# real-world-cryprography/APSU

Hardware: AMD Instinct MI355X
Metric: sender query-eval ms (ComputePowers + all BinBundles + gather), 16M-4096 params (lower is better)
Workload: dtype u64; 1 GPU; 16M-4096: n=8192, 4 bundle indices x 7 BinBundles (degrees [1303, 170]), 6 source -> 72 target powers, ps_low_degree=44; db_bytes_rank0=5459379072, binbundles_rank0=28, parallelism=binbundle-shard x1

## Files before the change

### apsu_amd/csrc/dev_consts.cpp

```cpp
#include "dev_consts.h"
#include "eval_plan.h"
#include "mac_core.h"

#include <algorithm>
#include <cstdint>
#include <cstdlib>
#include <cstring>
#include <stdexcept>
#include <string>
#include <utility>

namespace apsu_he {

uint32_t packed_row_bits(u64 q)
{
    const int bits = 64 - __builtin_clzll(q);
    for (u32 c = (u32)std::max(bits, 32); c < 64; c++) {
        u32 g = 2 * c, r = 32;
        while (r) { const u32 t2 = g % r; g = r; r = t2; }
        if ((32 - g) + 2 * c <= 128) return c;
    }
    return 64;
}

// ... 195 lines not shown
        DevLevel &d = dc.key_level[0];
        std::memset(&d, 0, sizeof(d));
        d.L = hp.K;
        for (int j = 0; j < hp.K; j++) d.q[j] = k.q[j];
    }
    for (u64 q : hp.key_q) {
        dc.max_multiple.push_back(~(u64)0 - (~(u64)0 % q) - 1);
        dc.row_bits.push_back(packed_row_bits(q));
    }
}

DeviceConstants build_device_constants(const HeParams &hp)
{
    DeviceConstants dc;
    build_transform_tables(hp, dc);
    build_levels(hp, dc);
    build_key(hp, dc);
    dc.data_primes_narrow = true;
    for (u64 q : hp.key_q) dc.data_primes_narrow = dc.data_primes_narrow && ntt_is_narrow(q, hp.logn);
    dc.ext_primes_narrow = dc.data_primes_narrow;
    for (u64 m : hp.aux_primes) dc.ext_primes_narrow = dc.ext_primes_narrow && ntt_is_narrow(m, hp.logn);
    dc.unlift_exact = hp.batching && hp.key_q[0] / 2 >= hp.t && hp.key_q[0] > 2 * hp.t;
    return dc;
}

EngineSwitches read_switches()
{
    EngineSwitches s;
    auto flag = [](const char *name, auto &out) { if (const char *v = std::getenv(name)) out = std::atoi(v) != 0; };
    auto size = [](const char *name, size_t &out) { if (const char *v = std::getenv(name)) out = std::strtoull(v, nullptr, 10); };
    flag("APSU_HE_SPLIT", s.two_stream_default);
    flag("APSU_HE_MAC_KARA", s.mac_kara);
    flag("APSU_HE_EVAL_SIDE", s.eval_side);
    flag("APSU_HE_PACKED_ROWS", s.packed_rows);
    flag("APSU_HE_EVAL_PER_TERM", s.force_per_term);
    flag("APSU_HE_SEED_EXPAND_HOST", s.seed_expand_host);
    flag("APSU_HE_FUSE_TAIL", s.fuse_tail);
    size("APSU_HE_EVAL_WS_BYTES", s.eval_ws_bytes);
    size("APSU_HE_ARENA_BYTES", s.arena_bytes);
    size("APSU_HE_NTT_LATENCY_LIMBS", s.ntt_latency_limbs);
    size("APSU_HE_SEED_REJ_CAP", s.seed_rej_cap);
    return s;
}

}
```

### apsu_amd/csrc/dev_consts.h

```cpp
#pragma once
#include <cstddef>
#include <vector>

#include "modmath.h"
#include "ntt_core.h"
#include "ntt_form.h"
#include "params.h"

namespace apsu_he {

constexpr int EW_T = 256;
constexpr int DMAXL = 8;
constexpr int DMAXB = DMAXL + 2;
constexpr int DMAXE = DMAXL + DMAXB;
constexpr u32 SEED_REJ_CAP = 8192;

struct ShoupConst { u64 w, wq; };

struct DevLevel {
    int L, nB, nBsk, E;
    Mod q[DMAXL];
    Mod bsk[DMAXB];
    Mod ext[DMAXE];
    u64 t;
// ... 65 lines not shown
}
inline NttTable make_ntt_table(const NttTablesHost &t, int logn, const TwPair *fwd, const TwPair *dit, const TwPair *scale)
{
    NttTable tb = make_ntt_table(t.mod.value, logn);
    tb.ninv = t.ninv;
    tb.ninv_q = t.ninv_q;
    tb.fwd = fwd;
    tb.dit = dit;
    tb.scale = scale;
    return tb;
}

struct DeviceConstants {
    std::vector<TwPair> tw;
    std::vector<NttTable> tabs;
    std::vector<ShoupConst> fin, drop, mdtw;
    std::vector<DevLevel> levels;
    DevKey key;
    std::vector<int> map_ext, map_ext_fin, map_ks, map_ksacc, map_ksacc_raw, map_ct;
    std::vector<DevLevel> key_level;
    std::vector<u64> max_multiple;
    bool data_primes_narrow = false;
    bool ext_primes_narrow = false;
    bool unlift_exact = false;
    std::vector<u32> row_bits;
    void relocate(const TwPair *tw_base, const ShoupConst *fin_base, const ShoupConst *drop_base, const ShoupConst *mdtw_base);
};
DeviceConstants build_device_constants(const HeParams &hp);

struct EngineSwitches {
    static constexpr size_t ARENA_AUTO = ~(size_t)0;
    int two_stream_default = -1;
    bool eval_side = true;
    bool packed_rows = true;
    size_t eval_ws_bytes = (size_t)6 << 30;
    size_t arena_bytes = ARENA_AUTO;
    bool force_per_term = false;
    int mac_kara = -1;
    bool seed_expand_host = false;
    size_t seed_rej_cap = SEED_REJ_CAP;
    bool fuse_tail = true;
    size_t ntt_latency_limbs = NTT_FORM_AUTO;
};
EngineSwitches read_switches();

}
```

### apsu_amd/csrc/emu/rules.cpp

```cpp
#include <cstring>
#include <set>
#include <stdexcept>
#include <vector>

#include "emu_common.h"
#include "bundle_layout.h"
#include "dev_consts.h"
#include "eval_plan.h"
#include "params.h"
#include "powers_dag.h"
#include "powers_sched.h"
#include "sched_policy.h"

using namespace apsu_he;

extern "C" {

const char *emu_last_error() { return g_err.c_str(); }

int emu_plan_walk(unsigned bits, int split_mode)
{
    WalkState s{};
    s.recycled = bits & 1; s.last_use_set = bits & 2; s.last_use_done = bits & 4; s.high_async = bits & 8; s.split_ok = bits & 16;
    s.prof_on = bits & 32; s.pipe_cp = bits & 64; s.force_pipe = bits & 128; s.inputs_ready = bits & 256; s.on_device = bits & 512;
    s.device_busy = bits & 1024; s.split_mode = split_mode;
    const WalkPlan p = plan_walk(s);
    return p.walk | (p.main_waits_high_ready ? 4 : 0) | (p.side_waits_last_use ? 8 : 0) | (p.side_waits_main ? 16 : 0) | (p.consumes_last_use ? 32 : 0);
}
int emu_pick_pooled_buffer(const unsigned char *entries, int count, int inputs_ready)
{
    std::vector<PoolEntryState> st(count);
    for (int i = 0; i < count; i++) st[i] = PoolEntryState{ (entries[i] & 1) != 0, (entries[i] & 2) != 0, (entries[i] & 4) != 0 };
    return pick_pooled_buffer(st.data(), st.size(), inputs_ready != 0);
}

int emu_plan_eval(unsigned bits, int low, int high, int L, int nB, uint32_t l, uint64_t q_last, uint64_t q_widest, int Bs, int max_terms)
{
    EvalState s{};
    s.low = low; s.high = high; s.L = L; s.nB = nB; s.l = l; s.q_last = q_last; s.q_widest = q_widest; s.Bs = Bs; s.max_terms = max_terms;
    s.high_in_flight = bits & 1; s.eval_side = bits & 2; s.prof_on = bits & 4; s.force_per_term = bits & 8; s.fuse_tensor = bits & 16;
    s.fuse_tail = bits & 32; s.lane2 = bits & 64; s.on_lane0 = bits & 128;
    const EvalPlan p = plan_eval(s);
    return (int)p.i0_fast | p.need_vlast << 1 | p.raw_drop << 2 | p.raw_i0 << 3 | p.fused_drop << 4 | p.summed << 5 | p.side << 6 | p.side_i0 << 7 |
           p.wait_high_ready << 8 | p.fuse_tensor << 9 | p.fuse_tail << 10 | p.cf << 11 | p.i0 << 13;
}
int emu_behz_unrolled(int L, int nB) { return behz_unrolled(L, nB); }

int emu_bundle_layout(uint32_t ps_low_degree, uint32_t degree, int first_chain_idx, uint64_t *out, int cap, uint32_t *where)
{
    try {
        const BundleLayout y = bundle_layout(ps_low_degree, degree, first_chain_idx);
        std::vector<u64> v{ y.use_ps, y.H, y.r, (u64)y.pt_level, y.ntt_count, y.lifted_count, y.runs.size() };
        for (const BundleRun &r : y.runs) v.insert(v.end(), { r.d0, r.count, (u64)r.kind, r.first_slot });
        for (size_t i = 0; i < v.size() && (int)i < cap; i++) out[i] = v[i];
        for (uint32_t d = 0; where && d <= degree; d++) { where[2 * d] = (uint32_t)y.where(d).kind; where[2 * d + 1] = y.where(d).slot; }
        return (int)v.size();
    } catch (const std::invalid_argument &e) { g_err = e.what(); return -1; }
}

void emu_ntt_form(int logn, int kind, size_t limbs, size_t latency_limbs, int narrow, int *out)
{
    const NttForm f = ntt_form(logn, (NttKind)kind, limbs, latency_limbs, narrow != 0);
    out[0] = f.threads; out[1] = f.coeffs_per_lane; out[2] = f.min_waves; out[3] = f.split;
}

int emu_params_info(const char *json, uint64_t *out, int cap)
{
    try {
        PSUParams p = PSUParams::Load(json);
        HeParams hp = HeParams::FromPSUParams(p);
        std::vector<u64> v;
        v.push_back(hp.n); v.push_back(hp.K); v.push_back(hp.first_chain_idx); v.push_back(hp.t);
        for (u64 q : hp.key_q) v.push_back(q);
        for (int j = 0; j < hp.K; j++) v.push_back(hp.ntt[j].psi);
        const LevelConstants &lv = hp.level[hp.first_chain_idx];
        v.push_back(lv.nB); v.push_back(lv.m_sk); v.push_back(lv.gamma);
        for (u64 b : lv.B) v.push_back(b);
// ... 166 lines not shown
```

### apsu_amd/csrc/engine.cpp

```cpp
#include "engine_impl.h"

namespace apsu_he {

void throw_hip(hipError_t e, const char *file, int line)
{
    throw HipError(std::string("HIP error: ") + hipGetErrorString(e) + " at " + file + ":" + std::to_string(line));
}

void DevBuf::alloc(size_t bytes)
{
    release();
    if (!bytes) return;
    HIP_CHECK(hipMalloc(&p_, bytes));
    bytes_ = bytes;
}
void DevBuf::release()
{
    if (p_) (void)hipFree(p_);
    p_ = nullptr;
    bytes_ = 0;
}

int Powers::slot_of(uint32_t bundle_idx) const
{
// ... 2 lines not shown
}

Engine::Engine(const HeParams &hp, const PSUParams *psu, int device) : hp_(hp), device_(device)
{
    if (psu) { psu_ = *psu; has_psu_ = true; }
    if (sw_.seed_rej_cap < 1 || sw_.seed_rej_cap > SEED_REJ_CAP) throw std::invalid_argument("APSU_HE_SEED_REJ_CAP outside 1 .. 8192");
    int ndev = 0;
    hipError_t e = hipGetDeviceCount(&ndev);
    if (e != hipSuccess || ndev == 0)
        throw HipError("no HIP device available: the query-evaluation engine has no CPU fallback");
    if (device < 0 || device >= ndev) throw std::invalid_argument("device index out of range");
    DeviceConstants dc = build_device_constants(hp_);
    data_primes_narrow_ = dc.data_primes_narrow;
    ext_primes_narrow_ = dc.ext_primes_narrow;
    unlift_exact_ = dc.unlift_exact;
    key_level_ = dc.key_level;
    max_multiple_ = dc.max_multiple;
    if (hp_.logn == 15) fuse_tensor_ = false;
    packed_rows_ = sw_.packed_rows && hp_.using_keyswitching;
    struct Restore { int prev = -1; ~Restore() { if (prev >= 0) (void)hipSetDevice(prev); } } restore;
    { int cur = -1; if (hipGetDevice(&cur) == hipSuccess && cur != device) restore.prev = cur; }
    HIP_CHECK(hipSetDevice(device));
    HIP_CHECK(hipStreamCreateWithFlags(&st_, hipStreamNonBlocking));
    {
        int least = 0, greatest = 0;
        HIP_CHECK(hipDeviceGetStreamPriorityRange(&least, &greatest));
        HIP_CHECK(hipStreamCreateWithPriority(&lanes_[1].st, hipStreamNonBlocking, greatest));
        HIP_CHECK(hipStreamCreateWithPriority(&lanes_[2].st, hipStreamNonBlocking, greatest));
    }
    HIP_CHECK(hipEventCreateWithFlags(&ev_main_, hipEventDisableTiming));
    HIP_CHECK(hipEventCreateWithFlags(&ev_fork_, hipEventDisableTiming));
    HIP_CHECK(hipEventCreateWithFlags(&ev_side_, hipEventDisableTiming));
    HIP_CHECK(hipEventCreateWithFlags(&ev_intt_, hipEventDisableTiming));

    auto each = [&](auto f) {
        f(d_tw_, dc.tw); f(d_tabs_, dc.tabs); f(d_fin_, dc.fin); f(d_drop_, dc.drop); f(d_levels_, dc.levels);
        f(d_map_ext_, dc.map_ext); f(d_map_ext_fin_, dc.map_ext_fin); f(d_map_ks_, dc.map_ks); f(d_map_ksacc_, dc.map_ksacc);
        f(d_map_ksacc_raw_, dc.map_ksacc_raw); f(d_map_ct_, dc.map_ct); f(d_mdtw_, dc.mdtw);
    };
    each([](DevBuf &b, const auto &v) { b.alloc(v.size() * sizeof(v[0])); });
    d_key_.alloc(sizeof(DevKey));
    dc.relocate(reinterpret_cast<const TwPair *>(d_tw_.p()), reinterpret_cast<const ShoupConst *>(d_fin_.p()),
                reinterpret_cast<const ShoupConst *>(d_drop_.p()), reinterpret_cast<const ShoupConst *>(d_mdtw_.p()));
    each([](DevBuf &b, const auto &v) { if (b.p()) HIP_CHECK(hipMemcpy(b.p(), v.data(), b.bytes(), hipMemcpyHostToDevice)); });
    HIP_CHECK(hipMemcpy(d_key_.p(), &dc.key, sizeof(DevKey), hipMemcpyHostToDevice));
    if (hp_.batching) {
        d_slot_map_.alloc(hp_.slot_map.size() * sizeof(uint32_t));
        HIP_CHECK(hipMemcpy(d_slot_map_.p(), hp_.slot_map.data(), hp_.slot_map.size() * sizeof(uint32_t), hipMemcpyHostToDevice));
    }
    if (has_psu_) {
        auto targets = create_powers_set(psu_.query_params.ps_low_degree, psu_.table_params.max_items_per_bin);
        if (!dag_.configure(psu_.query_params.query_powers, targets))
            throw std::invalid_argument("failed to configure PowersDag");
        const uint32_t ps = psu_.query_params.ps_low_degree;
        PowersScheds scheds = powers_scheds(dag_, ps);
        split_ok_ = scheds.split_ok;
        sched_ = std::move(scheds.all); sched_low_ = std::move(scheds.low); sched_high_ = std::move(scheds.high);
        sizes_ = power_sizes(sched_, hp_.using_keyswitching, dag_.depth());
        result_polys_ = apsu_he::result_polys(sizes_, ps, hp_.using_keyswitching, psu_.table_params.max_items_per_bin);
    }
    const size_t init = sw_.arena_bytes != EngineSwitches::ARENA_AUTO ? sw_.arena_bytes : 4096 * hp_.n * sizeof(u64);
    arena_.alloc(init);
    lanes_[1].arena.alloc(std::max<size_t>(init / 4, (size_t)1 << 20));
    lanes_[2].arena.alloc((size_t)1 << 20);
    stage_bytes_ = 4u << 20;
    HIP_CHECK(hipHostMalloc(&stage_, stage_bytes_));
    HIP_CHECK(hipHostMalloc(reinterpret_cast<void **>(&bad_source_), BAD_SLOTS * sizeof(unsigned)));
    for (int i = 0; i < BAD_SLOTS; i++) bad_source_[i] = 0;
}

Engine::~Engine()
{
    int cur = -1;
    const bool switched = hipGetDevice(&cur) == hipSuccess && cur != device_ && hipSetDevice(device_) == hipSuccess;
    struct Back { bool on; int dev; ~Back() { if (on) (void)hipSetDevice(dev); } } back{ switched, cur };
    if (st_) (void)hipStreamSynchronize(st_);
    for (Lane &l : lanes_) if (l.st) (void)hipStreamSynchronize(l.st);
    powers_pool_.clear();
    if (st_) (void)hipStreamDestroy(st_);
    for (Lane &l : lanes_) if (l.st) (void)hipStreamDestroy(l.st);
    for (hipEvent_t e : inflight_) if (e) (void)hipEventDestroy(e);
    for (PhaseSpan &sp : phase_spans_) for (hipEvent_t e : { sp.a, sp.b, sp.b2 }) if (e) (void)hipEventDestroy(e);
    for (hipEvent_t e : phase_pool_) if (e) (void)hipEventDestroy(e);
    for (hipEvent_t e : { query_start_, query_end_ }) if (e) (void)hipEventDestroy(e);
    if (ev_main_) (void)hipEventDestroy(ev_main_);
    for (OpClock &c : clock_) c.evs.release();
    if (ev_fork_) (void)hipEventDestroy(ev_fork_);
    if (ev_side_) (void)hipEventDestroy(ev_side_);
    if (ev_intt_) (void)hipEventDestroy(ev_intt_);
    if (stage_) (void)hipHostFree(stage_);
    if (bad_source_) (void)hipHostFree(bad_source_);
    if (wire_pinned_) (void)hipHostFree(wire_pinned_);
}

void Engine::wire_stage(size_t bytes, u64 **device, u64 **pinned)
{
    Enter g(this);
    if (wire_dev_.bytes() < bytes) { sync(); wire_dev_.alloc(bytes + bytes / 4); }
    if (wire_pinned_bytes_ < bytes) {
        sync();
        if (wire_pinned_) (void)hipHostFree(wire_pinned_);
        wire_pinned_ = nullptr; wire_pinned_bytes_ = 0;
        HIP_CHECK(hipHostMalloc(&wire_pinned_, bytes + bytes / 4));
        wire_pinned_bytes_ = bytes + bytes / 4;
    }
    *device = wire_dev_.u();
    *pinned = static_cast<u64 *>(wire_pinned_);
}

void Engine::sync()
{
    counters_[C_HOST_SYNC]++;
    HIP_CHECK(hipStreamSynchronize(st_));
    for (Lane &l : lanes_) if (l.st) HIP_CHECK(hipStreamSynchronize(l.st));
    if (prof_on_) prof_collect();
}

bool Engine::bad_source_pending(int slot, bool take)
{
    if (!bad_source_) return false;
    const unsigned v = *const_cast<volatile unsigned *>(bad_source_ + slot);
    if (v == bad_reported_[slot]) return false;
// ... 510 lines not shown
```

### apsu_amd/csrc/engine.h

```cpp
#pragma once
#include <hip/hip_runtime.h>

#include <functional>
#include <memory>
#include <mutex>
#include <string>
#include <vector>

#include "device.h"
#include "params.h"
#include "db_place.h"
#include "db_compact.h"
#include "bulk_place.h"
#include "powers_dag.h"
#include "powers_sched.h"
#include "bundle_layout.h"

namespace apsu_he {

struct HipError : std::runtime_error { using std::runtime_error::runtime_error; };

class DevBuf {
public:
    DevBuf() = default;
// ... 247 lines not shown
    const int *map_ksacc_raw(int chain_idx) const { return reinterpret_cast<const int *>(d_map_ksacc_raw_.p()) + chain_idx * (DMAXL + 1); }

    void d_ntt(u64 *data, size_t count, const int *modmap, int period, bool inverse, bool narrow);
    void d_ntt_ct(u64 *data, size_t polys, int chain_idx, bool inverse) { d_ntt(data, polys * (chain_idx + 1), map_ct(), chain_idx + 1, inverse, data_primes_narrow_); }
    bool d_relinearize(u64 *ct3, size_t ct_stride, int batch, const RelinKeys &rk, int chain_idx, u64 *ext_out = nullptr, int n_ext = 0,
                       u64 **defer_moddown = nullptr);
    void check_level(int chain_idx) const;
    void check_tier1_residues(const u64 *ct, size_t polys, int chain_idx, const char *what) const;
    void d_multiply_sized(const u64 *ea, int sa, const u64 *eb, int sb, u64 *out, int chain_idx);
    std::unique_ptr<Powers> compute_powers_nks(const uint32_t *bundle_indices, int nb, const u64 *const *src, bool on_device);
    void eval_bundles_nks(const Bundle *const *bundles, int count, const Powers &pw, const u64 *const *masks, bool masks_on_device,
                          u64 *out, bool out_on_device, u64 *const *out_rows);
    PowerSizes sizes_;
    uint32_t result_polys_ = 2;

    HeParams hp_;
    const EngineSwitches sw_ = read_switches();
    PSUParams psu_;
    bool has_psu_ = false;
    PowersDag dag_;
    int device_ = 0;
    hipStream_t st_ = nullptr;
    std::mutex mu_;

    DevBuf d_tabs_, d_tw_, d_levels_, d_key_, d_map_ct_, d_map_ext_, d_map_ext_fin_, d_map_ks_, d_map_ksacc_, d_map_ksacc_raw_, d_fin_, d_drop_, d_mdtw_;
    DevBuf arena_;
    size_t arena_off_ = 0;
    struct Lane { hipStream_t st = nullptr; DevBuf arena; size_t off = 0, job_seq = 0; };
    Lane lanes_[3];
    int cur_lane_ = 0, overflow_lane_ = 0;
    void switch_lane(int lane);
    hipEvent_t ev_main_ = nullptr;
    hipEvent_t ev_fork_ = nullptr, ev_side_ = nullptr, ev_intt_ = nullptr;
    bool inputs_ready_ = false;
    bool pipe_cp_ = true;
    bool force_pipe_ = false;
    bool data_primes_narrow_ = false;
    bool ext_primes_narrow_ = false;
    bool async_results_ = false;
    std::vector<hipEvent_t> inflight_;
    size_t inflight_head_ = 0, inflight_count_ = 0;
    int max_inflight_ = 2;
    void throttle_inflight();
    void mark_inflight();
    static constexpr int BAD_SLOTS = 16;
    unsigned *bad_source_ = nullptr;
    unsigned bad_reported_[BAD_SLOTS] = {};
    uint32_t query_seq_ = 0;
    void check_sources();
    void check_sources(const Powers &pw);
    bool bad_source_pending(int slot, bool take);
    void *stage_ = nullptr;
    size_t stage_bytes_ = 0, stage_off_ = 0;
    struct JobWay { DevBuf buf; std::vector<unsigned char> host; uint64_t stamp = 0; };
    struct JobSlot { JobWay way[4]; };
    uint64_t job_stamp_ = 0;
    std::vector<JobSlot> job_slots_;
    size_t job_seq_ = 0, job_seq_base_ = 0;
    std::vector<std::unique_ptr<Powers>> powers_pool_;
public:
    void recycle_powers(std::unique_ptr<Powers> p);
private:
    std::vector<DevBuf> retired_;
    uint64_t counters_[C_COUNT] = {};
    std::mutex wire_mu_;
    DevBuf wire_dev_;
// ... 1 lines not shown
    size_t wire_pinned_bytes_ = 0;

    PowersSched sched_, sched_low_, sched_high_;
    void mask_generate_impl(uint32_t count, u64 *masks_dev, u64 *values_host, u64 *blocks_host, const std::function<void(u64 *, size_t)> &fill);
    bool fuse_tensor_ = true;
    bool tier1_device_ = false;
    void tier1_done() { if (!tier1_device_ || prof_on_) sync(); }
    bool packed_rows_ = true;
    BundleLayout layout_of(uint32_t degree) const { return bundle_layout(psu_.query_params.ps_low_degree, degree, hp_.first_chain_idx); }
    std::unique_ptr<Bundle> new_bundle(uint32_t bundle_idx, uint32_t cache_idx, uint32_t degree, BundleLayout *layout = nullptr) const;
    size_t slot_bytes(int chain_idx, bool packed) const;
    void pack_bundle(Bundle &b);
    void unpack_bundle(Bundle &b);
    MacPlan plan_mac(const std::vector<MacStream> &streams, size_t nlimbs, size_t n) const;
    void d_mac(const MacPlan &p, const MacJob *jobs = nullptr);
    bool split_ok_ = false;
    int two_stream_mode_ = -1;
    struct DagRun;
    void dag_sources(DagRun &run, const u64 *const *src, bool on_device);
    void dag_level(DagRun &run, size_t d, const RelinKeys *rk);
    void dag_outputs(DagRun &run, Powers &pw, bool do_low, bool do_high);
    void dag_walk(const PowersSched &s, int nb, const u64 *const *src, bool on_device, const RelinKeys *rk, Powers &pw);
    void powers_header(Powers &pw, const uint32_t *bundle_indices, int nb, int low_level, int high_level);
    template <class F> void with_powers_span(F &&body);
    struct EvalCall;
    void eval_plain(EvalCall &c, const std::vector<int> &pl_ids);
    void eval_patstock(EvalCall &c, const std::vector<int> &ps_ids);
    void ps_cf_streams(const EvalCall &c, const PsBatch &g, std::vector<MacStream> &out);
    void ps_cf_mac(const EvalCall &c, const PsBatch &g);
    void ps_term_product(const EvalCall &c, const PsBatch &g);
    void ps_i0_finish(const EvalCall &c, const EvalPlan &plan, const PsBatch &g, u64 *i0);
    void ps_tables(EvalCall &c, const EvalPlan &plan, PsBatch &g);
    void ps_run(EvalCall &c, const EvalPlan &plan, PsBatch &g);
    void ps_mac(EvalCall &c, const EvalPlan &plan, PsBatch &g);
    void ps_side(EvalCall &c, const EvalPlan &plan, PsBatch &g);
    void ps_drop_ext(EvalCall &c, const EvalPlan &plan, PsBatch &g);
    void ps_products_summed(EvalCall &c, const EvalPlan &plan, PsBatch &g);
    void ps_products_per_term(EvalCall &c, const EvalPlan &plan, PsBatch &g);
    u64 *ps_i0(EvalCall &c, const EvalPlan &plan, PsBatch &g);
    void ps_epilogue(EvalCall &c, PsBatch &g, const u64 *i0);
    void finish_bundle(Bundle &b, const u64 *raw);
    void encode_bundle(Bundle &b, const u64 *poly);
    void decode_bundle(const Bundle &b, u64 *poly, u64 *coeff = nullptr);
    void decode_coeff(const Bundle &b, u64 *raw);
    void export_coeff(const Bundle &b, DevBuf &raw);
    void build_from_roots(Bundle &b, const u64 *droots, const uint32_t *dcounts, uint32_t bins, uint32_t stride);
    enum { NEED_PSU = 1, NEED_BATCHING, NEED_DECODE };
    void lookup_check(const char *what, int need = NEED_DECODE) const;
    u64 *decode_counted(const Bundle &b, uint32_t *dcounts, u64 *coeff = nullptr, EventStamps *evs = nullptr, size_t mid = 0);
    struct OpClock { EventStamps evs; double ms[OP_SPANS] = {}; } clock_[OP_COUNT];
    void lookup_impl(const Bundle *const *bundles, uint32_t n_bundles, const u64 *felts, const uint32_t *start, size_t count, uint32_t *counts,
                     unsigned char *flags);
    void eval_plain_queue(const Bundle *const *bundles, uint32_t n_bundles, const u64 *const *xs, const u64 *const *masks, u64 *out, unsigned char *is_bin,
                          u32 *bad, EventStamps &evs, size_t first);
    static void eval_plain_collect(const EventStamps &evs, size_t first, uint32_t n_bundles, double *ms);
    struct BinsCounted { u64 *poly, *coeff; uint32_t *dcounts; const uint32_t *counts; };
    struct BinsFound { std::vector<uint32_t> occ, found, mult; std::vector<u64> hits; uint32_t hstride = 0; };
    bool bins_prepare(const Bundle &b, int form);
    BinsCounted bins_counted(const Bundle &b, bool want_coeff, uint32_t *counts, EventStamps &evs);
    void bins_search(const BinsCounted &c, bool kernel, const uint32_t *stride, EventStamps &evs, size_t s, BinsFound &f);
    struct BinsDevice { uint32_t *occ, *found, *mult; u64 *hits; };
    BinsDevice bins_search_device(const BinsCounted &c, bool kernel, const uint32_t *stride, EventStamps &evs, size_t s, BinsFound &f);
    void bins_finish(const BinsCounted &c, BinsFound &f, u64 *roots, uint32_t stride);
    void keep_coeff_rows(const Bundle &b, const u64 *coeff, DevBuf &keep);
    void roots_tables();
    u64 roots_g_ = 0;
// ... 43 lines not shown
```

### apsu_amd/csrc/engine_eval.cpp

```cpp
#include "engine_impl.h"
#include "eval_plan.h"

namespace apsu_he {

static const u64 *bundle_slot(const Bundle &b, bool lifted, size_t slot, size_t dense_words)
{
    const DevBuf &buf = lifted ? b.lifted : b.ntt;
    if (!b.packed) return buf.u() + slot * dense_words;
    return reinterpret_cast<const u64 *>(static_cast<const char *>(buf.p()) + slot * (lifted ? b.lifted_slot_bytes : b.ntt_slot_bytes));
}
static u32 bundle_stride(const Bundle &b, bool lifted, size_t dense_words)
{
    return b.packed ? (u32)(lifted ? b.lifted_slot_bytes : b.ntt_slot_bytes) : (u32)dense_words;
}

struct Engine::EvalCall {
    const Bundle *const *bundles; const Powers &pw; const RelinKeys *rk;
    const u64 *const *masks; bool masks_on_device; u64 *const *out_rows;
    size_t n; uint32_t l; int high, low; size_t Ll, Lh, Eh; u32 low_term_stride;
    std::vector<int> bslot;
    int c0 = 0;
    u64 *res = nullptr, *mask_d = nullptr;
    const u64 *low_ptr(uint32_t power, int b) const { return pw.low.u() + (((size_t)b * pw.n_low + (power - 1)) * 2) * Ll * n; }
    const u64 *hext_ptr(uint32_t i, int b) const { return pw.hext.u() + (((size_t)b * pw.n_high + (i - 1)) * 2) * Eh * n; }
// ... 49 lines not shown
    }
}
void Engine::ps_cf_mac(const EvalCall &c, const PsBatch &g)
{
    std::vector<MacStream> cs;
    ps_cf_streams(c, g, cs);
    d_mac(plan_mac(cs, c.Lh, c.n));
}

void Engine::eval_patstock(EvalCall &c, const std::vector<int> &ps_ids)
{
    if (c.low < c.high) throw std::logic_error("the low powers lie below the high powers");
    PsBatch g;
    g.ids = ps_ids;
    std::stable_sort(g.ids.begin(), g.ids.end(), [&](int a, int b) { return c.slot(a) < c.slot(b); });
    g.Bs = (int)g.ids.size();
    g.nin.resize(g.Bs); g.in_off.resize(g.Bs);
    EvalState s{};
    for (int x = 0; x < g.Bs; x++) {
        const Bundle &b = c.bundle(g.ids[x]);
        g.nin[x] = (int)b.H - (b.r == 0 ? 1 : 0);
        g.in_off[x] = g.NI;
        g.NI += g.nin[x];
        s.max_terms = std::max(s.max_terms, g.nin[x]);
    }
    s.low = c.low; s.high = c.high;
    s.L = hlevel(c.high).L; s.nB = hlevel(c.high).nB;
    s.l = c.l; s.q_last = hlevel(c.low).q[c.Ll - 1];
    for (size_t j = 0; j < c.Lh; j++) s.q_widest = std::max(s.q_widest, hlevel(c.high).q[j]);
    s.Bs = g.Bs;
    s.high_in_flight = c.pw.high_async && c.pw.high_ready;
    s.eval_side = sw_.eval_side; s.prof_on = prof_on_; s.force_per_term = sw_.force_per_term; s.fuse_tensor = fuse_tensor_; s.fuse_tail = sw_.fuse_tail;
    s.lane2 = lanes_[2].st != nullptr; s.on_lane0 = cur_lane_ == 0;
    const EvalPlan plan = plan_eval(s);
    ps_tables(c, plan, g);
    ps_run(c, plan, g);
}

void Engine::ps_tables(EvalCall &c, const EvalPlan &plan, PsBatch &g)
{
    const size_t n = c.n, Ll = c.Ll, Lh = c.Lh;
    const uint32_t l = c.l;
    const int Bs = g.Bs;
    const bool cf_here = plan.cf == CF_WITH_MAC;
    const size_t w_inner = (size_t)g.NI * 2 * Ll * n, w_ssum = plan.i0_fast ? (size_t)Bs * 2 * Lh * n : 0;
    const size_t w_vlast = plan.need_vlast ? (size_t)Bs * l * 2 * n : 0, w_term = plan.i0_fast ? 0 : (size_t)Bs * l * 2 * Ll * n;
    const size_t w_cf = (size_t)Bs * 2 * Lh * n;
    g.inner = ws(w_inner + w_ssum + w_vlast + w_term + (cf_here ? w_cf : 0));
    g.ssum = g.inner + w_inner; g.vlast = g.ssum + w_ssum; g.term = g.vlast + w_vlast;
    g.cf = cf_here ? g.term + w_term : nullptr;
    std::vector<MacStream> ms;
    auto map_push = [&](size_t polys, int first_limb, int limbs) {
        for (size_t p = 0; p < polys; p++) for (int j = 0; j < limbs; j++) g.imap.push_back(first_limb + j);
    };
    for (int x = 0; x < Bs; x++) {
        const Bundle &b = c.bundle(g.ids[x]);
        for (int i = 1; i <= g.nin[x]; i++) {
            const u32 cnt = (u32)i < b.H ? l : b.r;
            ms.push_back(MacStream{ bundle_slot(b, false, (size_t)i * l, Ll * n), c.low_ptr(1, c.slot(g.ids[x])),
                                    g.inner + ((size_t)g.in_off[x] + i - 1) * 2 * Ll * n, cnt,
                                    bundle_stride(b, false, Ll * n), c.low_term_stride, (u32)(Ll * n), (u32)(Ll * n), 0, (u32)Ll,
                                    (u32)b.packed });
        }
    }
    map_push((size_t)g.NI * 2, 0, (int)Ll);
    if (plan.raw_drop) for (int &v : g.imap) v |= NTT_MAP_RAW;
// ... 5 lines not shown
                                    (u32)b.packed });
        }
        map_push((size_t)Bs * 2, 0, (int)Lh);
        if (plan.raw_i0) for (size_t x = g.imap.size() - (size_t)Bs * 2 * Lh; x < g.imap.size(); x++) g.imap[x] |= NTT_MAP_RAW;
    }
    std::vector<TermJob> tj;
    if (plan.need_vlast || !plan.i0_fast) {
        for (int x = 0; x < Bs; x++) {
            const Bundle &b = c.bundle(g.ids[x]);
            const int bs = c.slot(g.ids[x]);
            if (plan.i0_fast) {
                if (x == 0) g.term_packed = b.packed;
                else if (g.term_packed != (bool)b.packed) throw std::logic_error("BinBundles of one evaluation differ in their row format");
            }
            for (u32 j = 1; j <= l; j++) {
                if (plan.i0_fast)
                    tj.push_back(TermJob{ bundle_slot(b, false, j - 1, Ll * n), c.low_ptr(j, bs), g.vlast + ((size_t)x * l + j - 1) * 2 * n });
                else
                    ms.push_back(MacStream{ bundle_slot(b, false, j - 1, Ll * n), c.low_ptr(j, bs),
                                            g.term + ((size_t)x * l + j - 1) * 2 * Ll * n, 1, bundle_stride(b, false, Ll * n), c.low_term_stride,
                                            (u32)(Ll * n), (u32)(Ll * n), 0, (u32)Ll, (u32)b.packed });
            }
        }
        if (plan.i0_fast) {
            map_push((size_t)Bs * l * 2, (int)Ll - 1, 1);
            if (plan.raw_i0) for (size_t x = g.imap.size() - (size_t)Bs * l * 2; x < g.imap.size(); x++) g.imap[x] |= NTT_MAP_RAW;
        } else map_push((size_t)Bs * l * 2, 0, (int)Ll);
    }
    if (plan.side_i0) g.n_vlast_side = (size_t)Bs * l * 2;
    if (cf_here) { ps_cf_streams(c, g, ms); map_push((size_t)Bs * 2, 0, (int)Lh); }
    g.mac = plan_mac(ms, Ll, n);
    g.mac_jobs = upload_jobs(g.mac.jobs);
    if (!tj.empty()) { g.term_jobs = upload_jobs(tj); g.n_term = tj.size(); }
}

void Engine::ps_term_product(const EvalCall &c, const PsBatch &g)
{
    PROF(P_MAC, (uint64_t)g.n_term * (g.term_packed ? packed_row_bits(hp_.key_q[c.Ll - 1]) : 64));
    launch_term_product(dlevel(c.low), g.term_jobs, g.n_term, c.n, (int)c.Ll - 1, (u32)(c.Ll * c.n), (u32)c.n, g.term_packed, st_);
}
void Engine::ps_i0_finish(const EvalCall &c, const EvalPlan &plan, const PsBatch &g, u64 *i0)
{
    std::vector<I0Job> ij;
    for (int x = 0; x < g.Bs; x++)
        ij.push_back(I0Job{ g.ssum + (size_t)x * 2 * c.Lh * c.n, g.vlast + (size_t)x * c.l * 2 * c.n, i0 + (size_t)x * 2 * c.Lh * c.n, (int)c.l, 1 });
    PROFW(P_MODSWITCH, (size_t)g.Bs * c.n * (4 * c.Lh + 2 * c.l));
    launch_i0_finish(dlevel(c.low), upload_jobs(ij), c.n, g.Bs, st_, plan.raw_i0);
}

void Engine::ps_mac(EvalCall &c, const EvalPlan &plan, PsBatch &g)
{
    d_mac(g.mac, g.mac_jobs);
    g.imap_dev = upload_jobs(g.imap);
    if (plan.side_i0) HIP_CHECK(hipEventRecord(ev_fork_, st_));
    else if (g.n_term) ps_term_product(c, g);
    d_ntt(g.inner, g.imap.size() - g.n_vlast_side, g.imap_dev, (int)g.imap.size(), true, false);
    if (plan.side_i0) HIP_CHECK(hipEventRecord(ev_intt_, st_));
}

void Engine::ps_side(EvalCall &c, const EvalPlan &plan, PsBatch &g)
{
    g.cf = ws((size_t)g.Bs * 2 * c.Lh * c.n);
    if (plan.side_i0) g.i0_side = ws((size_t)g.Bs * 2 * c.Lh * c.n);
    else HIP_CHECK(hipEventRecord(ev_fork_, st_));
    switch_lane(2);
    struct Back { Engine *e; ~Back() { e->switch_lane(0); } } back{ this };
    HIP_CHECK(hipStreamWaitEvent(st_, ev_fork_, 0));
    if (plan.side_i0) {
        ps_term_product(c, g);
        d_ntt(g.vlast, g.n_vlast_side, g.imap_dev + (g.imap.size() - g.n_vlast_side), (int)g.n_vlast_side, true, false);
    }
    if (plan.wait_high_ready) HIP_CHECK(hipStreamWaitEvent(st_, c.pw.high_ready, 0));
    ps_cf_mac(c, g);
    d_ntt_ct(g.cf, (size_t)g.Bs * 2, c.high, true);
    if (plan.side_i0) {
        HIP_CHECK(hipStreamWaitEvent(st_, ev_intt_, 0));
        ps_i0_finish(c, plan, g, g.i0_side);
    }
    HIP_CHECK(hipEventRecord(ev_side_, st_));
}

void Engine::ps_drop_ext(EvalCall &c, const EvalPlan &plan, PsBatch &g)
{
    const size_t n = c.n;
    const int NI = g.NI;
    const LevelConstants &h = hlevel(c.high);
    g.ext = ws((size_t)NI * 2 * c.Eh * n);
    if (plan.fused_drop) {
        PROFW(P_BEHZ_EXT, (size_t)NI * 2 * n * (c.Ll + c.Eh));
        if (!launch_drop_behz_ext(dlevel(c.high), h.L, h.nB, g.inner, c.Ll * n, 1, g.ext, n, NI * 2, st_, plan.raw_drop))
            throw std::logic_error("the plan takes the fused drop + extension, the kernel table has none for this level");
    } else {
        u64 *innerh = g.inner;
        for (int lv = c.low; lv > c.high; lv--) {
            u64 *nxt = ws((size_t)NI * 2 * lv * n);
            { PROFW(P_MODSWITCH, (size_t)NI * 2 * n * (2 * lv + 1)); launch_modswitch(dlevel(lv), innerh, (size_t)2 * (lv + 1) * n, 2, nxt, n, NI, st_); }
            innerh = nxt;
        }
        { PROFW(P_BEHZ_EXT, (size_t)NI * 2 * n * (c.Lh + c.Eh)); launch_behz_ext(dlevel(c.high), h.L, h.nB, innerh, c.Lh * n, 1, g.ext, n, NI * 2, st_); }
    }
    d_ntt(g.ext, (size_t)NI * 2 * c.Eh, map_ext(c.high), (int)c.Eh, false, ext_primes_narrow_);
}

// ... 1 lines not shown
{
    const size_t n = c.n, Lh = c.Lh, Eh = c.Eh, nBskh = Eh - Lh;
    const int Bs = g.Bs, NI = g.NI;
    const LevelConstants &h = hlevel(c.high);
    const bool late_cf = plan.cf == CF_BEHIND_HIGH_READY;
    g.result = ws((size_t)Bs * 3 * Lh * n);
    u64 *dq = ws((size_t)NI * 3 * Lh * n + (size_t)Bs * 3 * nBskh * n + (late_cf ? (size_t)Bs * 2 * Lh * n : 0));
    u64 *bsum = dq + (size_t)NI * 3 * Lh * n;
    if (late_cf) {
        g.cf = bsum + (size_t)Bs * 3 * nBskh * n;
        ps_cf_mac(c, g);
    }
    std::vector<TensorSumJob> tj;
    std::vector<FinishSumJob> fj;
    std::vector<int> dmap;
    for (int x = 0; x < Bs; x++) {
        if (!g.nin[x]) { HIP_CHECK(hipMemsetAsync(g.result + (size_t)x * 3 * Lh * n, 0, 3 * Lh * n * sizeof(u64), st_)); continue; }
        const size_t job = (size_t)g.in_off[x];
        tj.push_back(TensorSumJob{ g.ext + job * 2 * Eh * n, c.hext_ptr(1, c.slot(g.ids[x])), dq + job * 3 * Lh * n,
                                   bsum + (size_t)x * 3 * nBskh * n, g.nin[x], 0 });
        fj.push_back(FinishSumJob{ dq + job * 3 * Lh * n, bsum + (size_t)x * 3 * nBskh * n, g.result + (size_t)x * 3 * Lh * n, g.nin[x], 0 });
    }
    const int rawf = behz_unrolled(h.L, h.nB) ? NTT_MAP_RAW : 0;
    for (size_t p = 0; p < (size_t)NI * 3; p++) for (size_t j = 0; j < Lh; j++) dmap.push_back((int)j | rawf);
    for (size_t p = 0; p < (size_t)Bs * 3; p++) for (size_t i = 0; i < nBskh; i++) dmap.push_back(hp_.bsk_id(h.nB, (int)i) | rawf);
    if (late_cf) for (size_t p = 0; p < (size_t)Bs * 2; p++) for (size_t j = 0; j < Lh; j++) dmap.push_back((int)j);
    if (plan.fuse_tensor) {
        std::vector<TensorJob> pj;
        for (int x = 0; x < Bs; x++)
            for (int i = 0; i < g.nin[x]; i++) {
                const size_t job = (size_t)g.in_off[x] + i;
                pj.push_back(TensorJob{ g.ext + job * 2 * Eh * n, c.hext_ptr(1 + i, c.slot(g.ids[x])), dq + job * 3 * Lh * n });
            }
        { PROFW(P_TENSOR, ((size_t)NI * 4 + (size_t)Bs * 3) * (Eh - Lh) * n); launch_tensor_sum(dlevel(c.high), (int)Eh, upload_jobs(tj), n, (int)tj.size(), (int)Lh, st_); }
        PROF(P_NTT_FUSED, dmap.size());
        launch_intt_tensor(hp_.logn, upload_jobs(pj), (int)pj.size(), (int)Lh, Eh * n, bsum, dmap.size() - pj.size() * 3 * Lh,
                           tabs(), upload_jobs(dmap), (int)dmap.size(), st_, sw_.ntt_latency_limbs);
    } else {
        { PROFW(P_TENSOR, ((size_t)NI * 4 * Eh + (size_t)NI * 3 * Lh + (size_t)Bs * 3 * (Eh - Lh)) * n); launch_tensor_sum(dlevel(c.high), (int)Eh, upload_jobs(tj), n, (int)tj.size(), 0, st_); }
        d_ntt(dq, dmap.size(), upload_jobs(dmap), (int)dmap.size(), true, false);
    }
    { PROFW(P_BEHZ_FINISH, ((size_t)NI * 3 * Lh + (size_t)Bs * 3 * (Eh - Lh) + (size_t)Bs * 3 * Lh) * n); launch_behz_finish_sum(dlevel(c.high), h.L, h.nB, upload_jobs(fj), n, (int)fj.size(), st_); }
}

void Engine::ps_products_per_term(EvalCall &c, const EvalPlan &plan, PsBatch &g)
{
    const size_t n = c.n, Lh = c.Lh, Eh = c.Eh;
    const int Bs = g.Bs, NI = g.NI;
    const LevelConstants &h = hlevel(c.high);
    g.result = ws((size_t)Bs * 3 * Lh * n);
    if (plan.cf == CF_BEHIND_HIGH_READY) {
        g.cf = ws((size_t)Bs * 2 * Lh * n);
        ps_cf_mac(c, g);
        d_ntt_ct(g.cf, (size_t)Bs * 2, c.high, true);
    }
    u64 *dbuf = ws((size_t)NI * 3 * Eh * n);
    u64 *tbuf = ws((size_t)NI * 3 * Lh * n);
    std::vector<TensorJob> tj;
    std::vector<FinishJob> fj;
    std::vector<SumJob> sj;
    for (int x = 0; x < Bs; x++) {
        for (int i = 1; i <= g.nin[x]; i++) {
            const size_t job = (size_t)g.in_off[x] + i - 1;
            tj.push_back(TensorJob{ g.ext + job * 2 * Eh * n, c.hext_ptr(i, c.slot(g.ids[x])), dbuf + job * 3 * Eh * n });
            fj.push_back(FinishJob{ dbuf + job * 3 * Eh * n, tbuf + job * 3 * Lh * n, 1, 0 });
        }
        sj.push_back(SumJob{ tbuf + (size_t)g.in_off[x] * 3 * Lh * n, g.result + (size_t)x * 3 * Lh * n, g.nin[x], 0 });
    }
    if (plan.fuse_tensor) {
        PROF(P_NTT_FUSED, tj.size() * 3 * Eh);
// ... 14 lines not shown
    if (plan.i0 == I0_SSUM) return g.ssum;
    u64 *i0 = nullptr;
    if (plan.i0 == I0_FINISH_MAIN) {
        i0 = ws((size_t)Bs * 2 * Lh * n);
        ps_i0_finish(c, plan, g, i0);
    } else {
        u64 *termh = g.term;
        for (int lv = c.low; lv > c.high; lv--) {
            u64 *nxt = ws((size_t)Bs * c.l * 2 * lv * n);
            { PROFW(P_MODSWITCH, (size_t)Bs * c.l * 2 * n * (2 * lv + 1)); launch_modswitch(dlevel(lv), termh, (size_t)2 * (lv + 1) * n, 2, nxt, n, Bs * (int)c.l, st_); }
            termh = nxt;
        }
        i0 = ws((size_t)Bs * 2 * Lh * n);
        HIP_CHECK(hipMemsetAsync(i0, 0, (size_t)Bs * 2 * Lh * n * sizeof(u64), st_));
        { PROF(P_OTHER, 0); launch_add_many(dlevel(c.high), i0, 2 * Lh * n, termh, (int)c.l, 2, n, Bs, st_); }
    }
    return i0;
}

void Engine::ps_epilogue(EvalCall &c, PsBatch &g, const u64 *i0)
{
    const size_t n = c.n, Lh = c.Lh;
    std::vector<EpiJob> ej;
    for (int x = 0; x < g.Bs; x++)
        ej.push_back(EpiJob{ g.result + (size_t)x * 3 * Lh * n, i0 + (size_t)x * 2 * Lh * n, g.cf + (size_t)x * 2 * Lh * n,
                             c.bundle(g.ids[x]).a0.u(), c.mask_ptr(g.ids[x]), c.res_ptr(g.ids[x]),
                             g.ks_acc ? g.ks_acc + (size_t)x * 2 * (Lh + 1) * n : nullptr });
    PROFW(P_MODSWITCH, (size_t)g.Bs * n * (7 * Lh + 4 + (g.ks_acc ? 2 * (Lh + 1) : 0)));
    launch_eval_epilogue(dlevel(0), c.high, upload_jobs(ej), Lh * n, hp_.irrelevant_bit_count, n, g.Bs, st_, g.ks_acc ? dkey() : nullptr);
}

void Engine::ps_run(EvalCall &c, const EvalPlan &plan, PsBatch &g)
{
    ps_mac(c, plan, g);
    if (plan.side) ps_side(c, plan, g);
    ps_drop_ext(c, plan, g);
    if (plan.wait_high_ready) HIP_CHECK(hipStreamWaitEvent(st_, c.pw.high_ready, 0));
    if (plan.summed) ps_products_summed(c, plan, g);
    else ps_products_per_term(c, plan, g);
    d_relinearize(g.result, 3 * c.Lh * c.n, g.Bs, *c.rk, c.high, nullptr, 0, plan.fuse_tail ? &g.ks_acc : nullptr);
    if (plan.side) HIP_CHECK(hipStreamWaitEvent(st_, ev_side_, 0));
    ps_epilogue(c, g, ps_i0(c, plan, g));
}

void Engine::eval_bundles(const Bundle *const *bundles, int count, const Powers &pw, const RelinKeys *rk,
                          const u64 *const *masks, bool masks_on_device, u64 *out, bool out_on_device, u64 *const *out_rows)
{
    if (out_rows && !out_on_device) throw std::invalid_argument("out_rows are device-accessible destinations");
    Enter g(this);
    if (!has_psu_) throw std::logic_error("context was created without PSUParams");
    if (count <= 0) return;
    const size_t n = hp_.n;
    job_seq_base_ = 256;
    if (pw.low_async && pw.high_ready) HIP_CHECK(hipStreamWaitEvent(st_, pw.high_ready, 0));
    struct LastUse {
        Engine *e; const Powers &p;
        ~LastUse()
        {
            if (e->cur_lane_ != 0) e->switch_lane(0);
            if (!p.last_use && hipEventCreateWithFlags(&p.last_use, hipEventDisableTiming) != hipSuccess) { p.last_use = nullptr; p.last_use_set = false; return; }
            p.last_use_set = hipEventRecord(p.last_use, e->st_) == hipSuccess;
        }
    } last_use_mark{ this, pw };
    PhaseSpan ev_span;
    if (phase_on_) { ev_span.phase = PH_PROCESS_BIN_BUNDLE_CACHE; ev_span.a = phase_event(st_); }
    const uint32_t ps = psu_.query_params.ps_low_degree, l = ps;
// ... 77 lines not shown
```

### apsu_amd/csrc/eval_plan.h

```cpp
#pragma once
#include <cstddef>
#include <cstdint>

namespace apsu_he {

constexpr bool behz_unrolled(int L, int nB) { return L == nB && L <= 3; }

struct EvalState {
    int low, high;
    int L, nB;
    uint32_t l;
    uint64_t q_last;
    uint64_t q_widest;
    int Bs, max_terms;
    bool high_in_flight;
    bool eval_side, prof_on, force_per_term, fuse_tensor, fuse_tail;
    bool lane2, on_lane0;
};
enum CfPlace {
    CF_WITH_MAC = 0,
    CF_SIDE_LANE = 1,
    CF_BEHIND_HIGH_READY = 2
};
enum I0Form {
    I0_SIDE = 0,
    I0_SSUM = 1,
    I0_FINISH_MAIN = 2,
    I0_GENERAL = 3
};
struct EvalPlan {
    bool i0_fast, need_vlast, raw_drop, raw_i0, fused_drop, summed, side, side_i0, wait_high_ready, fuse_tensor, fuse_tail;
    int cf;
    int i0;
};

inline EvalPlan plan_eval(const EvalState &s)
{
    EvalPlan p{};
    const int Lh = s.high + 1;
    p.i0_fast = (s.low - s.high <= 1) && ((unsigned __int128)(s.l + 1) * s.q_last < ((unsigned __int128)1 << 64));
    p.need_vlast = p.i0_fast && s.low > s.high;
    p.raw_drop = s.low == s.high + 1 && behz_unrolled(s.L, s.nB);
    p.raw_i0 = p.need_vlast;
    p.fused_drop = p.raw_drop;
    p.wait_high_ready = s.high_in_flight;
    p.side = s.eval_side && s.high_in_flight && !s.prof_on && p.i0_fast && s.low != s.high && s.lane2 && s.on_lane0;
    p.side_i0 = p.side && (size_t)s.Bs * s.l <= 4096;
    p.cf = !s.high_in_flight ? CF_WITH_MAC : p.side ? CF_SIDE_LANE : CF_BEHIND_HIGH_READY;
    p.i0 = p.side_i0 ? I0_SIDE : p.i0_fast && s.low == s.high ? I0_SSUM : p.i0_fast ? I0_FINISH_MAIN : I0_GENERAL;
    p.summed = !s.force_per_term && Lh <= 4 && (unsigned __int128)s.max_terms * s.q_widest < ((unsigned __int128)1 << 63);
    p.fuse_tensor = s.fuse_tensor;
    p.fuse_tail = s.fuse_tail;
    return p;
}

}
```

Baseline: 3.210 ms.

## Fork side-lane i0 terms before MAC and overlap bsum tensor/NTT on side stream

Adds two default-on plan options. side_early launches the side-lane term product and vlast NTT before the main MAC instead of after it, so they overlap the MAC. side_bsum splits the fused tensor-sum plus INTT so that the Bsk-base tensor sum and NTT run on lane 2 while the main stream runs the q-part INTT, joined by an event. This adds stream forks, events and extra job uploads, and concurrent kernels may compete for compute units.

```diff
diff --git a/apsu_amd/csrc/dev_consts.cpp b/apsu_amd/csrc/dev_consts.cpp
--- a/apsu_amd/csrc/dev_consts.cpp
+++ b/apsu_amd/csrc/dev_consts.cpp
@@ -251,6 +251,8 @@
     flag("APSU_HE_SPLIT", s.two_stream_default);
     flag("APSU_HE_MAC_KARA", s.mac_kara);
     flag("APSU_HE_EVAL_SIDE", s.eval_side);
+    flag("APSU_HE_SIDE_EARLY", s.side_early);
+    flag("APSU_HE_SIDE_BSUM", s.side_bsum);
     flag("APSU_HE_PACKED_ROWS", s.packed_rows);
     flag("APSU_HE_EVAL_PER_TERM", s.force_per_term);
     flag("APSU_HE_SEED_EXPAND_HOST", s.seed_expand_host);
diff --git a/apsu_amd/csrc/dev_consts.h b/apsu_amd/csrc/dev_consts.h
--- a/apsu_amd/csrc/dev_consts.h
+++ b/apsu_amd/csrc/dev_consts.h
@@ -121,6 +121,8 @@
     static constexpr size_t ARENA_AUTO = ~(size_t)0;
     int two_stream_default = -1;
     bool eval_side = true;
+    bool side_early = true;
+    bool side_bsum = true;
     bool packed_rows = true;
     size_t eval_ws_bytes = (size_t)6 << 30;
     size_t arena_bytes = ARENA_AUTO;
diff --git a/apsu_amd/csrc/emu/rules.cpp b/apsu_amd/csrc/emu/rules.cpp
--- a/apsu_amd/csrc/emu/rules.cpp
+++ b/apsu_amd/csrc/emu/rules.cpp
@@ -39,10 +39,10 @@
     EvalState s{};
     s.low = low; s.high = high; s.L = L; s.nB = nB; s.l = l; s.q_last = q_last; s.q_widest = q_widest; s.Bs = Bs; s.max_terms = max_terms;
     s.high_in_flight = bits & 1; s.eval_side = bits & 2; s.prof_on = bits & 4; s.force_per_term = bits & 8; s.fuse_tensor = bits & 16;
-    s.fuse_tail = bits & 32; s.lane2 = bits & 64; s.on_lane0 = bits & 128;
+    s.fuse_tail = bits & 32; s.lane2 = bits & 64; s.on_lane0 = bits & 128; s.side_early = bits & 256; s.side_bsum = bits & 512;
     const EvalPlan p = plan_eval(s);
     return (int)p.i0_fast | p.need_vlast << 1 | p.raw_drop << 2 | p.raw_i0 << 3 | p.fused_drop << 4 | p.summed << 5 | p.side << 6 | p.side_i0 << 7 |
-           p.wait_high_ready << 8 | p.fuse_tensor << 9 | p.fuse_tail << 10 | p.cf << 11 | p.i0 << 13;
+           p.wait_high_ready << 8 | p.fuse_tensor << 9 | p.fuse_tail << 10 | p.cf << 11 | p.i0 << 13 | p.side_i0_early << 15 | p.side_bsum << 16;
 }
 int emu_behz_unrolled(int L, int nB) { return behz_unrolled(L, nB); }
 
diff --git a/apsu_amd/csrc/engine.cpp b/apsu_amd/csrc/engine.cpp
--- a/apsu_amd/csrc/engine.cpp
+++ b/apsu_amd/csrc/engine.cpp
@@ -58,6 +58,8 @@
     HIP_CHECK(hipEventCreateWithFlags(&ev_fork_, hipEventDisableTiming));
     HIP_CHECK(hipEventCreateWithFlags(&ev_side_, hipEventDisableTiming));
     HIP_CHECK(hipEventCreateWithFlags(&ev_intt_, hipEventDisableTiming));
+    HIP_CHECK(hipEventCreateWithFlags(&ev_bfork_, hipEventDisableTiming));
+    HIP_CHECK(hipEventCreateWithFlags(&ev_bjoin_, hipEventDisableTiming));
 
     auto each = [&](auto f) {
         f(d_tw_, dc.tw); f(d_tabs_, dc.tabs); f(d_fin_, dc.fin); f(d_drop_, dc.drop); f(d_levels_, dc.levels);
@@ -114,6 +116,8 @@
     if (ev_fork_) (void)hipEventDestroy(ev_fork_);
     if (ev_side_) (void)hipEventDestroy(ev_side_);
     if (ev_intt_) (void)hipEventDestroy(ev_intt_);
+    if (ev_bfork_) (void)hipEventDestroy(ev_bfork_);
+    if (ev_bjoin_) (void)hipEventDestroy(ev_bjoin_);
     if (stage_) (void)hipHostFree(stage_);
     if (bad_source_) (void)hipHostFree(bad_source_);
     if (wire_pinned_) (void)hipHostFree(wire_pinned_);
diff --git a/apsu_amd/csrc/engine.h b/apsu_amd/csrc/engine.h
--- a/apsu_amd/csrc/engine.h
+++ b/apsu_amd/csrc/engine.h
@@ -303,6 +303,7 @@
     void switch_lane(int lane);
     hipEvent_t ev_main_ = nullptr;
     hipEvent_t ev_fork_ = nullptr, ev_side_ = nullptr, ev_intt_ = nullptr;
+    hipEvent_t ev_bfork_ = nullptr, ev_bjoin_ = nullptr;
     bool inputs_ready_ = false;
     bool pipe_cp_ = true;
     bool force_pipe_ = false;
@@ -370,6 +371,8 @@
     void ps_i0_finish(const EvalCall &c, const EvalPlan &plan, const PsBatch &g, u64 *i0);
     void ps_tables(EvalCall &c, const EvalPlan &plan, PsBatch &g);
     void ps_run(EvalCall &c, const EvalPlan &plan, PsBatch &g);
+    void ps_side_i0_terms(const EvalCall &c, const PsBatch &g);
+    void ps_side_early(EvalCall &c, PsBatch &g);
     void ps_mac(EvalCall &c, const EvalPlan &plan, PsBatch &g);
     void ps_side(EvalCall &c, const EvalPlan &plan, PsBatch &g);
     void ps_drop_ext(EvalCall &c, const EvalPlan &plan, PsBatch &g);
diff --git a/apsu_amd/csrc/engine_eval.cpp b/apsu_amd/csrc/engine_eval.cpp
--- a/apsu_amd/csrc/engine_eval.cpp
+++ b/apsu_amd/csrc/engine_eval.cpp
@@ -105,6 +105,7 @@
     s.high_in_flight = c.pw.high_async && c.pw.high_ready;
     s.eval_side = sw_.eval_side; s.prof_on = prof_on_; s.force_per_term = sw_.force_per_term; s.fuse_tensor = fuse_tensor_; s.fuse_tail = sw_.fuse_tail;
     s.lane2 = lanes_[2].st != nullptr; s.on_lane0 = cur_lane_ == 0;
+    s.side_early = sw_.side_early; s.side_bsum = sw_.side_bsum;
     const EvalPlan plan = plan_eval(s);
     ps_tables(c, plan, g);
     ps_run(c, plan, g);
@@ -176,6 +177,7 @@
     g.mac = plan_mac(ms, Ll, n);
     g.mac_jobs = upload_jobs(g.mac.jobs);
     if (!tj.empty()) { g.term_jobs = upload_jobs(tj); g.n_term = tj.size(); }
+    g.imap_dev = upload_jobs(g.imap);
 }
 
 void Engine::ps_term_product(const EvalCall &c, const PsBatch &g)
@@ -192,11 +194,27 @@
     launch_i0_finish(dlevel(c.low), upload_jobs(ij), c.n, g.Bs, st_, plan.raw_i0);
 }
 
+void Engine::ps_side_i0_terms(const EvalCall &c, const PsBatch &g)
+{
+    ps_term_product(c, g);
+    d_ntt(g.vlast, g.n_vlast_side, g.imap_dev + (g.imap.size() - g.n_vlast_side), (int)g.n_vlast_side, true, false);
+}
+
+void Engine::ps_side_early(EvalCall &c, PsBatch &g)
+{
+    g.cf = ws((size_t)g.Bs * 2 * c.Lh * c.n);
+    g.i0_side = ws((size_t)g.Bs * 2 * c.Lh * c.n);
+    HIP_CHECK(hipEventRecord(ev_fork_, st_));
+    switch_lane(2);
+    struct Back { Engine *e; ~Back() { e->switch_lane(0); } } back{ this };
+    HIP_CHECK(hipStreamWaitEvent(st_, ev_fork_, 0));
+    ps_side_i0_terms(c, g);
+}
+
 void Engine::ps_mac(EvalCall &c, const EvalPlan &plan, PsBatch &g)
 {
     d_mac(g.mac, g.mac_jobs);
-    g.imap_dev = upload_jobs(g.imap);
-    if (plan.side_i0) HIP_CHECK(hipEventRecord(ev_fork_, st_));
+    if (plan.side_i0) { if (!plan.side_i0_early) HIP_CHECK(hipEventRecord(ev_fork_, st_)); }
     else if (g.n_term) ps_term_product(c, g);
     d_ntt(g.inner, g.imap.size() - g.n_vlast_side, g.imap_dev, (int)g.imap.size(), true, false);
     if (plan.side_i0) HIP_CHECK(hipEventRecord(ev_intt_, st_));
@@ -204,15 +222,16 @@
 
 void Engine::ps_side(EvalCall &c, const EvalPlan &plan, PsBatch &g)
 {
-    g.cf = ws((size_t)g.Bs * 2 * c.Lh * c.n);
-    if (plan.side_i0) g.i0_side = ws((size_t)g.Bs * 2 * c.Lh * c.n);
-    else HIP_CHECK(hipEventRecord(ev_fork_, st_));
+    if (!plan.side_i0_early) {
+        g.cf = ws((size_t)g.Bs * 2 * c.Lh * c.n);
+        if (plan.side_i0) g.i0_side = ws((size_t)g.Bs * 2 * c.Lh * c.n);
+        else HIP_CHECK(hipEventRecord(ev_fork_, st_));
+    }
     switch_lane(2);
     struct Back { Engine *e; ~Back() { e->switch_lane(0); } } back{ this };
-    HIP_CHECK(hipStreamWaitEvent(st_, ev_fork_, 0));
-    if (plan.side_i0) {
-        ps_term_product(c, g);
-        d_ntt(g.vlast, g.n_vlast_side, g.imap_dev + (g.imap.size() - g.n_vlast_side), (int)g.n_vlast_side, true, false);
+    if (!plan.side_i0_early) {
+        HIP_CHECK(hipStreamWaitEvent(st_, ev_fork_, 0));
+        if (plan.side_i0) ps_side_i0_terms(c, g);
     }
     if (plan.wait_high_ready) HIP_CHECK(hipStreamWaitEvent(st_, c.pw.high_ready, 0));
     ps_cf_mac(c, g);
@@ -280,10 +299,30 @@
                 const size_t job = (size_t)g.in_off[x] + i;
                 pj.push_back(TensorJob{ g.ext + job * 2 * Eh * n, c.hext_ptr(1 + i, c.slot(g.ids[x])), dq + job * 3 * Lh * n });
             }
-        { PROFW(P_TENSOR, ((size_t)NI * 4 + (size_t)Bs * 3) * (Eh - Lh) * n); launch_tensor_sum(dlevel(c.high), (int)Eh, upload_jobs(tj), n, (int)tj.size(), (int)Lh, st_); }
-        PROF(P_NTT_FUSED, dmap.size());
-        launch_intt_tensor(hp_.logn, upload_jobs(pj), (int)pj.size(), (int)Lh, Eh * n, bsum, dmap.size() - pj.size() * 3 * Lh,
-                           tabs(), upload_jobs(dmap), (int)dmap.size(), st_, sw_.ntt_latency_limbs);
+        if (plan.side_bsum) {
+            const size_t n_q = pj.size() * 3 * Lh, n_b = (size_t)Bs * 3 * nBskh;
+            const std::vector<int> qmap(dmap.begin(), dmap.begin() + n_q), bmap(dmap.begin() + n_q, dmap.begin() + n_q + n_b);
+            const TensorSumJob *tj_dev = upload_jobs(tj);
+            const TensorJob *pj_dev = upload_jobs(pj);
+            const int *qmap_dev = upload_jobs(qmap), *bmap_dev = upload_jobs(bmap);
+            HIP_CHECK(hipEventRecord(ev_bfork_, st_));
+            {
+                switch_lane(2);
+                struct Back { Engine *e; ~Back() { e->switch_lane(0); } } back{ this };
+                HIP_CHECK(hipStreamWaitEvent(st_, ev_bfork_, 0));
+                { PROFW(P_TENSOR, ((size_t)NI * 4 + (size_t)Bs * 3) * (Eh - Lh) * n); launch_tensor_sum(dlevel(c.high), (int)Eh, tj_dev, n, (int)tj.size(), (int)Lh, st_); }
+                d_ntt(bsum, n_b, bmap_dev, (int)n_b, true, false);
+                HIP_CHECK(hipEventRecord(ev_bjoin_, st_));
+            }
+            PROF(P_NTT_FUSED, n_q);
+            launch_intt_tensor(hp_.logn, pj_dev, (int)pj.size(), (int)Lh, Eh * n, nullptr, 0, tabs(), qmap_dev, (int)n_q, st_, sw_.ntt_latency_limbs);
+            HIP_CHECK(hipStreamWaitEvent(st_, ev_bjoin_, 0));
+        } else {
+            { PROFW(P_TENSOR, ((size_t)NI * 4 + (size_t)Bs * 3) * (Eh - Lh) * n); launch_tensor_sum(dlevel(c.high), (int)Eh, upload_jobs(tj), n, (int)tj.size(), (int)Lh, st_); }
+            PROF(P_NTT_FUSED, dmap.size());
+            launch_intt_tensor(hp_.logn, upload_jobs(pj), (int)pj.size(), (int)Lh, Eh * n, bsum, dmap.size() - pj.size() * 3 * Lh,
+                               tabs(), upload_jobs(dmap), (int)dmap.size(), st_, sw_.ntt_latency_limbs);
+        }
     } else {
         { PROFW(P_TENSOR, ((size_t)NI * 4 * Eh + (size_t)NI * 3 * Lh + (size_t)Bs * 3 * (Eh - Lh)) * n); launch_tensor_sum(dlevel(c.high), (int)Eh, upload_jobs(tj), n, (int)tj.size(), 0, st_); }
         d_ntt(dq, dmap.size(), upload_jobs(dmap), (int)dmap.size(), true, false);
@@ -364,6 +403,7 @@
 
 void Engine::ps_run(EvalCall &c, const EvalPlan &plan, PsBatch &g)
 {
+    if (plan.side_i0_early) ps_side_early(c, g);
     ps_mac(c, plan, g);
     if (plan.side) ps_side(c, plan, g);
     ps_drop_ext(c, plan, g);
diff --git a/apsu_amd/csrc/eval_plan.h b/apsu_amd/csrc/eval_plan.h
--- a/apsu_amd/csrc/eval_plan.h
+++ b/apsu_amd/csrc/eval_plan.h
@@ -16,6 +16,7 @@
     bool high_in_flight;
     bool eval_side, prof_on, force_per_term, fuse_tensor, fuse_tail;
     bool lane2, on_lane0;
+    bool side_early, side_bsum;
 };
 enum CfPlace {
     CF_WITH_MAC = 0,
@@ -30,6 +31,8 @@
 };
 struct EvalPlan {
     bool i0_fast, need_vlast, raw_drop, raw_i0, fused_drop, summed, side, side_i0, wait_high_ready, fuse_tensor, fuse_tail;
+    bool side_i0_early;
+    bool side_bsum;
     int cf;
     int i0;
 };
@@ -51,6 +54,8 @@
     p.summed = !s.force_per_term && Lh <= 4 && (unsigned __int128)s.max_terms * s.q_widest < ((unsigned __int128)1 << 63);
     p.fuse_tensor = s.fuse_tensor;
     p.fuse_tail = s.fuse_tail;
+    p.side_i0_early = p.side_i0 && s.side_early;
+    p.side_bsum = p.side && p.summed && p.fuse_tensor && s.side_bsum;
     return p;
 }
 
```

New measurement: 3.269 ms. +1.9%, slower.
